# danshapero/sigma

Hardware: AMD Instinct MI355X
Metric: SpMV GB/s (achieved HBM) + CG iters/sec on 5-pt Laplacian, N=1e7 (higher is better)
Workload: dtype f64; 1 GPU; 5-point 2D Poisson CSR, 3162x3162 rows per GPU (rank 0: n=9998244, nnz=49978572), fp64 SpMV y=A*x; rows_per_gpu=9998244, nnz_per_gpu=49978572, parallelism=row-partition x1, matrix_resident_bytes_per_gpu=479920788, reference_layout_bytes_per_gpu=639735844, full=False

## Files before the change

include/sigma_hip.h:

```cpp
#ifndef SIGMA_HIP_H
#define SIGMA_HIP_H

#include <stddef.h>
#include <stdint.h>

#ifdef __cplusplus
extern "C" {
#endif

typedef struct sgm_mat_s *sgm_mat;
typedef struct sgm_pc_s *sgm_pc;
typedef struct sgm_solver_s *sgm_solver;
typedef struct sgm_comm_s *sgm_comm;

enum {
    SGM_OK = 0,
    SGM_ERR_BAD_ARG = 1,
    SGM_ERR_DIMS = 2,
    SGM_ERR_HIP = 3,
    SGM_ERR_RCCL = 4,
    SGM_ERR_NOT_CONVERGED = 5,
    SGM_ERR_NO_DEVICE = 6,
    SGM_ERR_ALLOC = 7,
    SGM_ERR_UNSUPPORTED = 8
// ... 50 lines not shown
int sgm_mat_get_entries(sgm_mat A, int64_t m, const int32_t *i, const int32_t *j, double *z_out, int where);
int sgm_mat_zero(sgm_mat A);
int sgm_mat_scalar_multiply(sgm_mat A, double alpha);
int sgm_mat_add_matrix(sgm_mat A, sgm_mat B, const double *alpha_or_null);
int sgm_edit_plan_create(sgm_edit_plan *out, sgm_mat A, int64_t m, const int32_t *i, const int32_t *j, int where);
int sgm_edit_plan_apply(sgm_edit_plan plan, sgm_mat A, const double *z, int mode, int zero_first, int where);
int sgm_edit_plan_info(sgm_edit_plan plan, int64_t *out4);
int sgm_edit_plan_destroy(sgm_edit_plan plan);
int sgm_edit_locate_host(int32_t nrow, int32_t ncol, const int32_t *ptr_1based, const int32_t *node_1based, int64_t m,
                         const int32_t *i, const int32_t *j, int64_t *hit_off, int32_t *hit_slot, int64_t capacity,
                         int64_t *needed, int64_t *first_missing);
int sgm_composite_create(sgm_mat *out, int32_t nrb, int32_t ncb, const int32_t *row_ptr_1based,
                         const int32_t *col_ptr_1based, const sgm_mat *blocks);
int sgm_mat_info(sgm_mat A, int32_t *nrow, int32_t *ncol, int64_t *nnz, int32_t *fmt,
                 int64_t *x_len );
int sgm_graph_bfs_order(sgm_mat A, int32_t *p_out);
int sgm_graph_greedy_coloring(sgm_mat A, int32_t *colors_out, int32_t *num_colors);
int sgm_graph_greedy_color_order(sgm_mat A, int32_t *p_out, int32_t *ptrs_out, int32_t ptrs_len,
                                 int32_t *num_colors);
int sgm_mat_left_permute(sgm_mat A, const int32_t *p, int where);
int sgm_mat_right_permute(sgm_mat A, const int32_t *p, int where);
int sgm_mat_kernel(sgm_mat A, char *buf, int len);
int sgm_mat_footprint(sgm_mat A, int64_t *resident_bytes, int64_t *matvec_bytes);
int sgm_mat_destroy(sgm_mat A);

int sgm_dot(int64_t n, const double *a, const double *b, double *result, int where);
int sgm_axpy(int64_t n, double alpha, const double *x, double *y, int where);

int sgm_pc_create(sgm_pc *out, int32_t kind );
int sgm_jacobi_create(sgm_pc *out, sgm_mat A);
int sgm_ildu0_create(sgm_pc *out, sgm_mat A);
int sgm_pc_setup(sgm_pc pc, sgm_mat A);
int sgm_pc_apply(sgm_pc pc, const double *r, double *z, int where);
int sgm_pc_get(sgm_pc pc, const char *name, void *out_host, size_t bytes, size_t *needed);
int sgm_pc_info(sgm_pc pc, int32_t part, int32_t *out4, double *est_us, char *path_name, int len);
int sgm_pc_destroy(sgm_pc pc);

int sgm_mg_create(sgm_pc *out, int32_t ncoarse, const sgm_mat *P ,
                  double omega, int32_t nu_pre, int32_t nu_post, int32_t coarse_sweeps);
int sgm_mg_level_matrix(sgm_pc pc, int32_t level, sgm_mat *borrowed);

int sgm_cg_create(sgm_solver *out, double tolerance);
int sgm_bicgstab_create(sgm_solver *out, double tolerance);
int sgm_gmres_create(sgm_solver *out, double tolerance, int32_t restart);
int sgm_solver_setup(sgm_solver s, sgm_mat A);
int sgm_solver_set_max_iter(sgm_solver s, int64_t max_iter );
// ... 64 lines not shown
```

sigma_amd/__init__.py:

```python
from __future__ import annotations

import ctypes as C
import os

import numpy as np

_HERE = os.path.dirname(os.path.abspath(__file__))
LIB_PATH = os.path.join(_HERE, "libsigma_hip.so")

SGM_HOST, SGM_DEVICE = 0, 1
FMT_CSR, FMT_ELL = 1, 2

_lib = None


class SigmaError(RuntimeError):

    def __init__(self, code, msg):
        super().__init__(f"[sigma_hip status {code}] {msg}")
        self.code = code


def build(force=False):
    import subprocess
# ... 198 lines not shown
        _ck(lib().sgm_graph_greedy_color_order(self._h, p.ctypes.data_as(C.c_void_p), ptrs.ctypes.data_as(C.c_void_p),
                                               C.c_int32(len(ptrs)), C.byref(nc)))
        return p, ptrs[:nc.value + 1].copy(), nc.value

    def left_permute(self, p):
        pp, w, _k = _arg(p, np.int32)
        _ck(lib().sgm_mat_left_permute(self._h, pp, C.c_int(w)))

    def right_permute(self, p):
        pp, w, _k = _arg(p, np.int32)
        _ck(lib().sgm_mat_right_permute(self._h, pp, C.c_int(w)))

    def set_option(self, name, value):
        if hasattr(self, "_build"):
            self._build()
        _ck(lib().sgm_mat_set_option(self._h, name.encode(), C.c_int(int(value))))
        return self

    @property
    def kernel(self):
        buf = C.create_string_buffer(64)
        _ck(lib().sgm_mat_kernel(self._h, buf, C.c_int(64)))
        return buf.value.decode()

    def set_solver(self, solver):
        self.solver = solver
        solver.setup(self)

    def set_preconditioner(self, pc):
        self.pc = pc
        pc.setup(self)

    def solve(self, x, b):
        if self.solver is None:
            raise SigmaError(1, "A%solve: no solver set (linear_operator_interface.f90:213-233)")
        return self.solver.solve(self, x, b, self.pc)

    def get(self, name, dtype):
        need = C.c_size_t(0)
        _ck(lib().sgm_mat_get(self._h, name.encode(), None, C.c_size_t(0), C.byref(need)))
        out = np.zeros(need.value // np.dtype(dtype).itemsize, dtype)
        _ck(lib().sgm_mat_get(self._h, name.encode(), C.c_void_p(out.ctypes.data), C.c_size_t(out.nbytes), None))
        return out

    def _triples(self, i, j, z=None):
        if not (_is_torch(i) or _is_torch(j) or (z is not None and _is_torch(z))):
# ... 831 lines not shown
```

sigma_amd/csrc/sgm_internal.hpp:

```cpp
#pragma once
#include <hip/hip_runtime.h>

#include <cstdarg>
#include <cstdint>
#include <cstdio>
#include <cstring>
#include <string>
#include <atomic>
#include <utility>
#include <vector>

#include "../../include/sigma_hip.h"

namespace sgm {

extern std::string g_err;
int fail(int code, const char *fmt, ...);

#define SGM_HIP(call)                                                              \
    do {                                                                           \
        hipError_t e__ = (call);                                                   \
        if (e__ != hipSuccess)                                                     \
            return sgm::fail(SGM_ERR_HIP, "%s:%d: %s -> %s", __FILE__, __LINE__,   \
                             #call, hipGetErrorString(e__));                       \
// ... 95 lines not shown
inline int vec_grid(int64_t n)
{
    int64_t g = (n + 4 * kBlock - 1) / (4 * kBlock);
    if (g < 1) g = 1;
    if (g > 2048) g = 2048;
    return (int)g;
}

struct ScalarRef {
    const double *ptr;
    int count;
};

struct HaloNbr {
    int peer = -1;
    int32_t send_count = 0;
    int32_t *send_idx = nullptr;
    double *send_buf = nullptr;
    int32_t recv_offset = 0;
    int32_t recv_count = 0;
};

struct SliceSched { int32_t *tab = nullptr; int32_t lo = 0, hi = 0, grid = 0, iters = 0, band = 0; };

struct Part {
    MatOptions opt = g_opt.mat;
    int32_t n = 0;
    int32_t ncol_own = 0;
    int32_t n_halo = 0;
    int32_t int_lo = 0, int_hi = 0;
    int64_t nnz = 0;
    int64_t row_begin = 0;
    int32_t *rowptr = nullptr;
    int32_t *col = nullptr;
    double *val = nullptr;
    uint8_t *code = nullptr;
    int32_t *dict = nullptr;
    int32_t ndict = 0;
    int32_t dict_reach = 0;
    int32_t max_row = 0;
    double *sval = nullptr;
    uint32_t *scode = nullptr;
    int32_t *scol = nullptr;
    uint8_t *sbcode = nullptr;
    bool lean = false;
    double *sl_val = nullptr;
    int32_t *sl_col = nullptr;
    uint16_t *sl_perm = nullptr;
    int64_t *sl_off = nullptr;
    int64_t sl_total = 0;
    int32_t *sl_win0 = nullptr;
    int32_t sl_gs = 1;
    int32_t sl_span = 0;
    int32_t sw = 0;
    int32_t sched_period = 0;
    mutable SliceSched sched[3];
    mutable int nsched = 0;
    const int32_t *run_sched = nullptr;
    int32_t run_iters = 0;
    int32_t max_d = 0;
    int32_t *ecol = nullptr;
    double *eval = nullptr;
    int32_t *edeg = nullptr;
    uint8_t *ecode = nullptr;
    int32_t emdp = 0;
    int32_t *cb_perm = nullptr;
    double *cb_sval = nullptr;
    uint16_t *cb_lcol = nullptr;
    int32_t *cb_bstart = nullptr;
    uint16_t *cb_lpos = nullptr;
    void *cb_fdesc = nullptr;
    double *cb_P = nullptr;
    int32_t cb_cols = 0, cb_nb = 0, cb_R = 0, cb_ntiles = 0, cb_chunks = 0;
    int32_t cb_maxd = 0;
    int64_t cb_count = 0;
    double col_spread = -1.0;
    std::vector<HaloNbr> nbrs;
    double *xext = nullptr;
    int dot_grid_override = 0;
    int64_t xlen() const { return (int64_t)ncol_own + n_halo; }
};

// ... 81 lines not shown
struct SpmvDots {
    const double *const *w = nullptr;
    double *const *part_wy = nullptr;
    double *const *part_yy = nullptr;
};
int spmv_parts(sgm_mat A, const double *const *x, double *const *y, bool add,
               const SpmvDots *dots, const int *flag_done, int *grid_out, int gen = 0x7fffffff,
               bool chain = false, bool halo_ready = false);

int build_csr_part(Part &p, int32_t n, int32_t ncol_own, int32_t n_halo, int64_t nnz,
                   const int32_t *ptr1, const int32_t *node1, const double *val, int where, bool validate = true);
int clone_csr_plain(sgm_mat A, sgm_mat *out);
int color_order_device(sgm_mat A, int32_t **dp, std::vector<int32_t> &ptrs);
int diag_block_plain(const Part &p, sgm_mat *out);
void part_kernel_name(const Part &p, int fmt, char *name, size_t len);
int permuted_part(const Part &p, const int32_t *p1_dev, Part &q, const int32_t *hmap_dev = nullptr,
                  const std::vector<int32_t *> *send_order = nullptr);
int halo_attach_order(const Part &p, const int32_t *p1_dev, const std::vector<std::pair<int32_t, int32_t>> &segments,
                      std::vector<int32_t> &hmap_host);
int exchange_halo_orders(sgm_mat A, const std::vector<int32_t> &mine, std::vector<int32_t *> &out);
int spmv_grid(const Part &p, bool whole = false);
int matvec_plain(sgm_mat A, const double *x, double *y);
int csr_need_arrays(const Part &p);
int ensure_transpose(sgm_mat A);
void csr_release_arrays(const Part &p);

struct Slab3;
int slab3_build(Slab3 **out, int32_t n, const std::vector<int32_t> &Lptr, const std::vector<int32_t> &Lnode,
                const std::vector<int32_t> &Uptr, const std::vector<int32_t> &Unode, const int32_t *dLptr, const int32_t *dLnode,
                const int32_t *dUptr, const int32_t *dUnode);
int slab3_refresh(Slab3 *S, const double *Lval, const double *Uval, const double *D);
void slab3_apply(const Slab3 *S, const double *r, double *z, const int *flag, int spin_limit, int32_t *sticky);
void slab3_lower_result(const Slab3 *S, double *dst);
int slab_dims_device(int32_t n, const int32_t *dptr, const int32_t *dnode, bool lower, int32_t *w, int32_t *h);
void slab3_dims(const Slab3 *S, int32_t *w, int32_t *h);
int slab3_aborted(const Slab3 *S, int32_t *abL, int32_t *abU);
void slab3_info(const Slab3 *S, int32_t out[6]);
int slab3_clocks(const Slab3 *S, std::vector<long long> &out);
void slab3_free(Slab3 *S);

}

#if defined(__HIPCC__)
namespace sgm {

template <int CTRL>
// ... 114 lines not shown
```

sigma_amd/csrc/sgm_layouts.hip:

```cpp
#include "sgm_spmv_select.hpp"

namespace sgm {

__global__ void k_dec1(int32_t *a, int64_t n)
{
    int64_t i = (int64_t)blockIdx.x * blockDim.x + threadIdx.x;
    const int64_t stride = (int64_t)gridDim.x * blockDim.x;
    for (; i < n; i += stride) a[i] -= 1;
}

__global__ void k_check_ptr1(const int32_t *__restrict__ ptr1, int64_t n, int64_t nnz, unsigned long long *bad)
{
    int64_t i = (int64_t)blockIdx.x * blockDim.x + threadIdx.x;
    const int64_t stride = (int64_t)gridDim.x * blockDim.x;
    for (; i <= n; i += stride) {
        const int32_t a = ptr1[i];
        bool ok = true;
        if (i == 0) ok = a == 1;
        if (i < n) ok = ok && ptr1[i + 1] >= a;
        else ok = ok && (int64_t)a - 1 == nnz;
        if (!ok) atomicMin(bad, (unsigned long long)i);
    }
}

// ... 237 lines not shown
        hipLaunchKernelGGL(k_sl_unpack, dim3((unsigned)std::min<int64_t>(((int64_t)p.n + 255) / 256, 4096)), dim3(256), 0, st, p.n, p.sw,
                           (const int32_t *)p.rowptr, (const uint32_t *)p.scode, (const int32_t *)p.dict, (const double *)p.sval,
                           mk_col ? p.col : nullptr, mk_val ? p.val : nullptr, mk_code ? p.code : nullptr);
    SGM_HIP(hipGetLastError());
    SGM_HIP(hipStreamSynchronize(st));
    return SGM_OK;
}
int lean_val_buffer(Part &p)
{
    if (!p.lean || p.val) return SGM_OK;
    SGM_TRY(dalloc(&p.val, (size_t)p.nnz + 2));
    SGM_HIP(hipMemsetAsync(p.val + p.nnz, 0, 2 * sizeof(double), g_rt.stream));
    return SGM_OK;
}
void csr_release_arrays(const Part &cp)
{
    Part &p = const_cast<Part &>(cp);
    if (!p.lean || !lean_applies(p)) return;
    (void)hipStreamSynchronize(g_rt.stream);
    dfree(p.val); dfree(p.col); dfree(p.code);
    p.val = nullptr; p.col = nullptr; p.code = nullptr;
}

int pack_sliced(Part &p)
{
    if (p.sl_val && p.n > 0) {
        const int64_t nch = (((int64_t)p.n + kSlRows - 1) / kSlRows) * (kSlRows / kSellChunk);
        hipLaunchKernelGGL(k_sell_fill, dim3((unsigned)std::min<int64_t>((nch + 3) / 4, 65536)), dim3(256), 0, g_rt.stream, p.n,
                           (const int32_t *)p.rowptr, (const int32_t *)nullptr, (const double *)p.val, (const int64_t *)p.sl_off,
                           (const uint16_t *)p.sl_perm, (int32_t *)nullptr, p.sl_val);
        SGM_HIP(hipGetLastError());
    }
    if ((!p.scode && !p.scol && !p.sbcode) || p.n == 0) return SGM_OK;
    const int64_t nsl = ((int64_t)p.n + kSlRows - 1) / kSlRows;
    if (p.ecol)
        hipLaunchKernelGGL(k_sl_pack_ell, dim3((unsigned)std::min<int64_t>(nsl, 65536)), dim3(256), 0, g_rt.stream, p.n, p.sw,
                           p.max_d, (const double *)p.eval, p.sval);
    else
        hipLaunchKernelGGL(k_sl_pack, dim3((unsigned)std::min<int64_t>(nsl, 65536)), dim3(256), 0, g_rt.stream, p.n, p.sw,
                           (const int32_t *)p.rowptr, (const double *)p.val, p.sval);
    SGM_HIP(hipGetLastError());
    return SGM_OK;
}

__global__ void k_fill32(int64_t n, int32_t *a, int32_t v)
{
    int64_t i = (int64_t)blockIdx.x * blockDim.x + threadIdx.x;
    const int64_t stride = (int64_t)gridDim.x * blockDim.x;
    for (; i < n; i += stride) a[i] = v;
}

constexpr int kDictSlots = 1024;
constexpr int32_t kDictEmpty = INT32_MIN;
__global__ __launch_bounds__(256) void k_dict_collect(int32_t n, const int32_t *__restrict__ rowptr, const int32_t *__restrict__ col,
                                                      int32_t *table, int *count, int *max_row)
{
    constexpr int kLocal = 512;
    __shared__ int32_t ltab[kLocal];
    __shared__ int lcount;
    for (int t = threadIdx.x; t < kLocal; t += 256) ltab[t] = kDictEmpty;
    if (threadIdx.x == 0) lcount = 0;
    __syncthreads();
    int mr = 0;
    int32_t mine[8];
// ... 226 lines not shown
                           reinterpret_cast<int32_t *>(p.scode), (int32_t)-1);
        p.sw = W;
    }
    hipLaunchKernelGGL(k_dict_encode, dim3(grid), dim3(256), 0, st, n, (const int32_t *)p.rowptr, (const int32_t *)p.col,
                       (const int32_t *)p.dict, p.ndict, p.code, sliced ? p.scode : nullptr);
    SGM_HIP(hipGetLastError());
    if (sliced) SGM_TRY(pack_sliced(p));
    int Wb = 0;
#define PICK(WW) if (!Wb && p.max_row <= WW) Wb = WW;
    SGM_SLB_WIDTHS(PICK)
#undef PICK
    const int Wc = (Wb + 7) / 8 * 8;
    if (!sliced && p.opt.csr_sliced && Wb && p.ndict <= 255 && p.max_row > 8 && (double)Wb * n <= 1.35 * (double)nnz) {
        rows_padded = ((size_t)n + kSlRows - 1) / kSlRows * kSlRows;
        SGM_TRY(dalloc(&p.sbcode, rows_padded * Wc));
        SGM_TRY(dalloc(&p.sval, rows_padded * Wb));
        p.sw = Wb;
        hipLaunchKernelGGL(k_slb_pack_codes, dim3((unsigned)std::min<size_t>(rows_padded / kSlRows, 65536)), dim3(256), 0, st, n, Wb,
                           (const int32_t *)p.rowptr, (const uint8_t *)p.code, p.sbcode);
        SGM_HIP(hipGetLastError());
        SGM_TRY(pack_sliced(p));
    }
    SGM_HIP(hipStreamSynchronize(st));
    if (p.scode || p.sbcode) SGM_TRY(detect_sched_period_csr(p, dict));
    if (!p.scode && !p.sbcode) {
        SGM_TRY(build_sell(p));
        if (p.sl_val) {
            dfree(p.code); dfree(p.dict);
            p.code = nullptr; p.dict = nullptr;
            p.ndict = 0; p.dict_reach = 0;
        }
    }
    csr_go_lean(p);
    return SGM_OK;
}

__global__ __launch_bounds__(256) void k_ell_dict_collect(int32_t n, int32_t max_d, const int32_t *__restrict__ ecol, int32_t *table,
                                                          int *count)
{
    constexpr int kLocal = 512;
    __shared__ int32_t ltab[kLocal];
    __shared__ int lcount;
    for (int t = threadIdx.x; t < kLocal; t += 256) ltab[t] = kDictEmpty;
    if (threadIdx.x == 0) lcount = 0;
    __syncthreads();
    int32_t mine[8];
// ... 197 lines not shown
    int rc = dalloc(&q.rowptr, (size_t)p.n + 1);
    if (rc == SGM_OK) rc = dalloc(&q.col, (size_t)p.nnz + 4);
    if (rc == SGM_OK) rc = dalloc(&q.val, (size_t)p.nnz + 2);
    if (rc != SGM_OK) { sgm_mat_destroy(C); return rc; }
    (void)hipMemcpyAsync(q.rowptr, p.rowptr, ((size_t)p.n + 1) * 4, hipMemcpyDeviceToDevice, st);
    (void)hipMemsetAsync(q.col + p.nnz, 0, 16, st);
    (void)hipMemsetAsync(q.val + p.nnz, 0, 16, st);
    if (p.nnz) {
        (void)hipMemcpyAsync(q.col, p.col, (size_t)p.nnz * 4, hipMemcpyDeviceToDevice, st);
        (void)hipMemcpyAsync(q.val, p.val, (size_t)p.nnz * 8, hipMemcpyDeviceToDevice, st);
    }
    if (hipStreamSynchronize(st) != hipSuccess || hipGetLastError() != hipSuccess) { sgm_mat_destroy(C); return fail(SGM_ERR_HIP, "clone_csr_plain: copy failed"); }
    *out = C;
    return SGM_OK;
}

int rebuild_csr_formats(Part &p)
{
    SGM_TRY(csr_need_arrays(p));
    p.lean = false;
    dfree(p.code); dfree(p.dict); dfree(p.sval); dfree(p.scode); dfree(p.scol); dfree(p.sbcode);
    p.code = nullptr; p.dict = nullptr; p.sval = nullptr; p.scode = nullptr; p.scol = nullptr; p.sbcode = nullptr;
    free_sell(p);
    free_ell_colblock(p);
    p.ndict = 0; p.dict_reach = 0; p.sw = 0; p.max_row = 0; p.sched_period = 0;
    free_slice_sched(p);
    return build_offset_dict(p, nullptr, nullptr);
}
int rebuild_ell_formats(Part &p)
{
    dfree(p.ecode); dfree(p.dict); dfree(p.sval); dfree(p.scode);
    p.ecode = nullptr; p.dict = nullptr; p.dict_reach = 0; p.emdp = 0; p.sval = nullptr; p.scode = nullptr; p.sw = 0; p.sched_period = 0;
    free_slice_sched(p);
    SGM_TRY(build_ell_offset_dict(p));
    SGM_TRY(build_ell_colblock(p));
    return refresh_ell_colblock_values(p);
}
int sgm_invalidate_transpose(sgm_mat A)
{
    if (A->T) { sgm_mat_destroy(A->T); A->T = nullptr; }
    dfree(A->tperm);
    A->tperm = nullptr;
    A->t_stale = true;
    return SGM_OK;
}

void free_part(Part &p)
{
    dfree(p.rowptr); dfree(p.col); dfree(p.val); dfree(p.code); dfree(p.dict); dfree(p.sval); dfree(p.scode); dfree(p.scol); dfree(p.sbcode); dfree(p.ecol); dfree(p.eval); dfree(p.edeg); dfree(p.ecode); dfree(p.xext);
    for (auto &nb : p.nbrs) { dfree(nb.send_idx); dfree(nb.send_buf); }
    free_slice_sched(p);
    free_ell_colblock(p);
    free_sell(p);
    p = Part();
}

}
```

sigma_amd/csrc/sgm_mat.hip:

```cpp
#include "sgm_spmv_select.hpp"

namespace sgm {

struct Staged {
    double *dev = nullptr;
    bool owned = false;
    ~Staged() { if (owned) dfree(dev); }
};
int stage_in(Staged &s, const double *v, int64_t n, int where, bool copy)
{
    if (where == SGM_DEVICE && (reinterpret_cast<uintptr_t>(v) & 15) == 0) {
        s.dev = const_cast<double *>(v);
        return SGM_OK;
    }
    SGM_TRY(dalloc(&s.dev, (size_t)n));
    s.owned = true;
    if (copy)
        SGM_HIP(hipMemcpyAsync(s.dev, v, (size_t)n * 8,
                               where == SGM_HOST ? hipMemcpyHostToDevice : hipMemcpyDeviceToDevice,
                               g_rt.stream));
    return SGM_OK;
}
int stage_out(const Staged &s, double *v, int64_t n, int where)
{
// ... 371 lines not shown
    if (!mat_option_field(probe, name)) return fail(SGM_ERR_BAD_ARG, "sgm_mat_set_option: '%s' is not a matrix option", name);
    if (A->fmt == SGM_FMT_COMPOSITE) {
        for (sgm_mat_s *B : A->blocks)
            if (B) SGM_TRY(sgm_mat_set_option(B, name, value));
        return SGM_OK;
    }
    const bool cb_shape = !strcmp(name, "ell_colblock_cols") || !strcmp(name, "ell_colblock_rows");
    for (Part &p : A->parts) {
        int *f = mat_option_field(p.opt, name);
        const int old = *f;
        *f = v;
        if (old == v) continue;
        if ((p.ecol || (!p.lean && p.rowptr && p.col && p.val && p.n_halo == 0 && !p.sval && !p.sl_val)) &&
            (cb_shape || (!strcmp(name, "ell_colblock") && ((old != 0) != (v != 0) || v == 2 || old == 2)))) {
            SGM_TRY(build_ell_colblock(p));
            SGM_TRY(refresh_ell_colblock_values(p));
            SGM_HIP(hipStreamSynchronize(g_rt.stream));
        }
        if (!strcmp(name, "csr_lean") && !p.ecol) {
            if (v == 0) { SGM_TRY(csr_need_arrays(p)); p.lean = false; }
            else csr_go_lean(p);
        }
        if (!strcmp(name, "slice_sched")) free_slice_sched(p);
    }
    if (A->T) SGM_TRY(sgm_mat_set_option(A->T, name, value));
    return SGM_OK;
}

int sgm_mat_matvec(sgm_mat A, const double *x, double *y, int where)
{
    return matvec_impl(A, x, y, where, false);
}

int sgm_mat_matvec_add(sgm_mat A, const double *x, double *y, int where)
{
    return matvec_impl(A, x, y, where, true);
}

int sgm_composite_create(sgm_mat *out, int32_t nrb, int32_t ncb, const int32_t *row_ptr, const int32_t *col_ptr,
                         const sgm_mat *blocks)
{
    SGM_TRY(require_init());
    if (!out || nrb < 1 || ncb < 1 || !row_ptr || !col_ptr || !blocks)
        return fail(SGM_ERR_BAD_ARG, "sgm_composite_create: bad argument");
    sgm_mat A = new sgm_mat_s;
    A->fmt = SGM_FMT_COMPOSITE;
// ... 159 lines not shown
}
extern "C" {

int sgm_mat_kernel(sgm_mat A, char *buf, int len)
{
    if (!A || !buf || len < 1) return fail(SGM_ERR_BAD_ARG, "sgm_mat_kernel: bad argument");
    char name[64];
    if (A->fmt == SGM_FMT_COMPOSITE) snprintf(name, sizeof name, "composite");
    else part_kernel_name(A->parts[0], A->fmt, name, sizeof name);
    snprintf(buf, (size_t)len, "%s", name);
    return SGM_OK;
}

static int64_t part_resident_bytes(const Part &p)
{
    int64_t b = 0;
    const int64_t nsl = ((int64_t)p.n + kSlRows - 1) / kSlRows;
    if (p.rowptr) b += 4 * ((int64_t)p.n + 1);
    if (p.col) b += 4 * (p.nnz + 4);
    if (p.val) b += 8 * (p.nnz + 2);
    if (p.code) b += p.nnz + 16;
    if (p.dict) b += 4 * 256;
    if (p.sval) b += 8 * nsl * kSlRows * p.sw;
    if (p.scode) b += 4 * nsl * kSlRows;
    if (p.scol) b += 4 * nsl * kSlRows * p.sw;
    if (p.sbcode) b += nsl * kSlRows * ((p.sw + 7) / 8 * 8);
    if (p.sl_val) b += 12 * p.sl_total + 2 * nsl * kSlRows + 8 * (nsl * (kSlRows / kSellChunk) + 1);
    if (p.ecol) b += 4 * (int64_t)p.n * p.max_d;
    if (p.eval) b += 8 * (int64_t)p.n * p.max_d;
    if (p.edeg) b += 4 * (int64_t)p.n;
    if (p.ecode) b += (int64_t)p.n * p.emdp;
    if (p.xext) b += 8 * p.xlen();
    b += ell_colblock_resident_bytes(p);
    for (const auto &nb : p.nbrs) b += (int64_t)nb.send_count * (nb.send_buf ? 12 : 4);
    return b;
}
static int64_t part_matvec_bytes(const sgm_mat_s *A, const Part &p)
{
    const int64_t nsl = ((int64_t)p.n + kSlRows - 1) / kSlRows;
    int64_t m;
    if (A->fmt == SGM_FMT_ELL) {
        if (use_ell_colblock(p)) return ell_colblock_matvec_bytes(p);
        if (use_sliced_ell(p)) m = nsl * kSlRows * (8 * (int64_t)p.sw + 4);
        else if (p.ecode && p.opt.ell_offset_dict) m = (int64_t)p.n * (8 * (int64_t)p.max_d + p.emdp);
        else m = 12 * (int64_t)p.n * p.max_d;
    } else if (use_ell_colblock(p)) return ell_colblock_matvec_bytes(p);
    else if (use_sliced(p)) m = nsl * kSlRows * (8 * (int64_t)p.sw + 4);
    else if (use_slicedb(p)) m = nsl * kSlRows * (8 * (int64_t)p.sw + (p.sw + 7) / 8 * 8);
    else if (use_sliced32(p)) m = nsl * kSlRows * 12 * (int64_t)p.sw;
    else if (use_sell(p)) {
        m = 12 * p.sl_total + 2 * nsl * kSlRows + 8 * nsl * (kSlRows / kSellChunk);
        if (p.sl_win0 && p.opt.csr_xwindow)
            return m + ((nsl + p.sl_gs - 1) / p.sl_gs) * (8 * (int64_t)p.sl_span + 4) + 8 * (int64_t)p.n;
    }
    else if (use_offset_dict(p)) m = 9 * p.nnz + 4 * ((int64_t)p.n + 1);
    else m = 12 * p.nnz + 4 * ((int64_t)p.n + 1);
    return m + 8 * p.xlen() + 8 * (int64_t)p.n;
}

int sgm_mat_footprint(sgm_mat A, int64_t *resident_bytes, int64_t *matvec_bytes)
{
    if (!A) return fail(SGM_ERR_BAD_ARG, "sgm_mat_footprint: null matrix");
    int64_t res = 0, mv = 0;
    if (A->fmt == SGM_FMT_COMPOSITE) {
        for (sgm_mat C : A->blocks) {
            if (!C) continue;
            int64_t r = 0, m = 0;
            SGM_TRY(sgm_mat_footprint(C, &r, &m));
            mv += m + 8 * (int64_t)C->nrow;
        }
        mv += 8 * (int64_t)A->nrow;
    } else {
        for (const Part &p : A->parts) { res += part_resident_bytes(p); mv += part_matvec_bytes(A, p); }
        if (A->T) { int64_t r = 0; SGM_TRY(sgm_mat_footprint(A->T, &r, nullptr)); res += r + 4 * A->nnz; }
    }
    if (resident_bytes) *resident_bytes = res;
    if (matvec_bytes) *matvec_bytes = mv;
    return SGM_OK;
}

int sgm_mat_destroy(sgm_mat A)
{
    if (!A) return SGM_OK;
    for (auto &p : A->parts) free_part(p);
    if (A->T) sgm_mat_destroy(A->T);
    dfree(A->tperm);
    alg_plan_free(A->alg);
    delete A;
    return SGM_OK;
}

}
```

sigma_amd/csrc/sgm_runtime.hip:

```cpp
#include "sgm_internal.hpp"

#include <algorithm>

namespace sgm {

std::string g_err;
Runtime g_rt;
Options g_opt;
Heartbeat g_hb;
extern int g_force_collectives;

int fail(int code, const char *fmt, ...)
{
    char buf[1024];
    va_list ap;
    va_start(ap, fmt);
    vsnprintf(buf, sizeof buf, fmt, ap);
    va_end(ap);
    g_err = buf;
    return code;
}

bool trace_on()
{
// ... 69 lines not shown
    SGM_OPT(mat, ell_colblock_rows) SGM_OPT(mat, slice_sched) SGM_OPT(mat, coloring_pass)
    return nullptr;
}
int *solver_option_field(SolverOptions &o, const char *name)
{
    SGM_OPT(solver, cg_small) SGM_OPT(solver, bicgstab_small) SGM_OPT(solver, krylov_graph) SGM_OPT(solver, dot_order)
    SGM_OPT(solver, gmres_cgs2) SGM_OPT(solver, dist_halo_fused) SGM_OPT(solver, coop_spin_limit) SGM_OPT(solver, cg_coop_variant)
    SGM_OPT(solver, reorder_solve)
    return nullptr;
}
int *pc_option_field(PcOptions &o, const char *name)
{
    SGM_OPT(pc, ildu_strips) SGM_OPT(pc, ildu_rows) SGM_OPT(pc, pipeline_spin_limit) SGM_OPT(pc, ildu_reorder)
    return nullptr;
}
#undef SGM_OPT

int normalise_option(const char *name, int value, int *out)
{
    int v = value;
    if (!strcmp(name, "ell_colblock_cols")) v = std::min(kEllcbMaxCols, std::max(2, value)) & ~1;
    else if (!strcmp(name, "ell_colblock_rows")) v = value == 512 ? 512 : value == 256 ? 256 : 0;
    else if (!strcmp(name, "ildu_reorder")) v = value != 0;
    else if (!strcmp(name, "csr_sell")) v = value < 0 ? 0 : value > 2 ? 2 : value;
    else if (!strcmp(name, "csr_lean") || !strcmp(name, "csr_xwindow")) v = value != 0;
    else if (!strcmp(name, "slice_sched")) v = value <= 0 ? 0 : value == 1 ? 1 : std::max(4, value);
    else if (!strcmp(name, "krylov_graph")) v = value <= 0 ? 0 : value == 1 ? 1 : std::max(16, (value + 15) / 16 * 16);
    else if (!strcmp(name, "cg_small")) v = std::max(0, value);
    else if (!strcmp(name, "dist_halo_fused") || !strcmp(name, "reorder_solve")) v = value < 0 ? 0 : value > 2 ? 2 : value;
    else if (!strcmp(name, "coop_spin_limit")) v = std::max(0, value);
    else if (!strcmp(name, "gmres_cgs2")) v = value != 0;
    else if (!strcmp(name, "cg_coop_variant")) {
        const int r = value & 15;
        if (value < 0 || value > 31 || (r != 0 && r != 1 && r != 2 && r != 4 && r != 8))
            return fail(SGM_ERR_BAD_ARG, "option cg_coop_variant: rows per thread 0 (by size), 1, 2, 4 or 8, + 16 = no one-XCD variant");
    }
    else if (!strcmp(name, "coloring_pass")) v = value < 0 ? 0 : value > 2 ? 2 : value;
    else if (!strcmp(name, "pipeline_spin_limit")) v = std::max(0, value);
    else if (!strcmp(name, "dot_order") && value != 0 && value != 1)
        return fail(SGM_ERR_BAD_ARG, "option dot_order is 0 (tree) or 1 (the reference's sequential order)");
    *out = v;
    return SGM_OK;
}

}

// ... 121 lines not shown
```

sigma_amd/csrc/sgm_spmv.hip:

```cpp
#include "sgm_spmv_select.hpp"
#include "sgm_plan_host.hpp"

namespace sgm {




__device__ inline int64_t rowblock_of(int it, int b, int grid, int64_t nrb = 0, int mode = 1)
{
    const int per = grid >> 3;
    if (mode == 2) {
        const int64_t chunk = (nrb + 7) / 8;
        const int64_t local = (int64_t)it * per + (b >> 3);
        return local < chunk ? (int64_t)(b & 7) * chunk + local : nrb;
    }
    return (int64_t)it * grid + (int64_t)(b & 7) * per + (b >> 3);
}


template <class T>
__device__ inline T ld_stream(const T *p, bool nt)
{
    return nt ? __builtin_nontemporal_load(p) : *p;
}
// ... 329 lines not shown
#pragma unroll
                for (int u = 0; u < U; ++u)
                    if (u < cnt) z = z + vv[u] * xv[u];
                k += cnt;
            }
        }
        if (row < n) {
            const double yi = ADD ? (chain ? z : y0 + z) : 0.0 + z;
            __builtin_nontemporal_store(yi, y + row);
            if (DOT_W) dwy += w[row] * yi;
            if (DOT_YY) dyy += yi * yi;
        }
    }
    if (DOT_W) {
        const double t = block_sum<BLOCK>(dwy, red);
        if (tid == 0) part_wy[blockIdx.x] = t;
    }
    if (DOT_YY) {
        const double t = block_sum<BLOCK>(dyy, red);
        if (tid == 0) part_yy[blockIdx.x] = t;
    }
}

template <int W, bool ADD, bool DOT_W, bool DOT_YY>
__global__ __launch_bounds__(256) void k_csr_sl(
    int32_t n, const uint32_t *__restrict__ scode, const int32_t *__restrict__ dict,
    const double *__restrict__ sval, const double *__restrict__ x, double *__restrict__ y,
    const double *__restrict__ w, double *__restrict__ part_wy, double *__restrict__ part_yy,
    const int *__restrict__ flag_done, int gen, int remap, const int32_t *__restrict__ sched, int sched_iters)
{
    constexpr int BLOCK = 256;
    __shared__ int32_t dl[16];
    __shared__ double red[BLOCK / 64];
    const int st = flag_done ? *flag_done : 0;
    const int tid = threadIdx.x;
    const bool chain = (remap & 256) != 0;
    const int32_t dv = tid < 16 ? dict[tid] : 0;
    const int64_t nsl = ((int64_t)n + kSlRows - 1) / kSlRows;
    double dwy = 0.0, dyy = 0.0;

    int64_t first = blockIdx.x;
    if ((remap & 255) >= 3) {
        const int G = (remap & 255) == 3 ? 8 : (remap & 255) == 4 ? 2 : (remap & 255) == 6 ? 64 : (remap & 255) == 7 ? 128 : 32;
        const int xcd = blockIdx.x & 7, loc = blockIdx.x >> 3;
        first = (int64_t)(loc / G) * (8 * G) + xcd * G + loc % G;
    }
    int64_t sl = sched ? sched[blockIdx.x] : first;
    int sit = 0;
    u32x2 cw = {0xffffffffu, 0xffffffffu};
    f64x2 v[W];
    auto load_slice = [&](int64_t s_) {
        const int32_t row_ = (int32_t)(s_ * kSlRows) + 2 * tid;
        cw = __builtin_nontemporal_load(reinterpret_cast<const u32x2 *>(scode + row_));
        const f64x2 *vb = reinterpret_cast<const f64x2 *>(sval + s_ * (int64_t)(W * kSlRows)) + tid;
#pragma unroll
        for (int u = 0; u < W; ++u) v[u] = __builtin_nontemporal_load(vb + u * BLOCK);
// ... 521 lines not shown
    } while (0)
#define LV(B, T)                                \
    if (c.block == B && tile == T) {            \
        if (w && pyy) L(B, T, true, true);      \
        else if (w) L(B, T, true, false);       \
        else if (pyy) L(B, T, false, true);     \
        else L(B, T, false, false);             \
        return;                                 \
    }
    SGM_DO_VARIANTS(LV)
#undef LV
#undef L
}

template <bool ADD>
static void launch_csr_sl(const Part &p, int grid, const double *x, double *y, const double *w,
                          double *pwy, double *pyy, const int *flag, int gen)
{
    const SpmvCfg &c = spmv_cfg();
    hipStream_t st = g_rt.stream;
    int mode = c.remap == 1 ? ((grid <= kMaxGrid / 2 || (int64_t)p.n < (int64_t)32768 * kSlRows) ? 5 : 0) : (c.remap >= 3 ? c.remap : 0);
    if (mode >= 3 && grid % (8 * (mode == 3 ? 8 : mode == 4 ? 2 : mode == 6 ? 64 : mode == 7 ? 128 : 32)) != 0) mode = 0;
#define L(WW, DW, DY)                                                                                   \
    hipLaunchKernelGGL((k_csr_sl<WW, ADD, DW, DY>), dim3(grid), dim3(256), 0, st, p.n, p.scode, p.dict, \
                       p.sval, x, y, w, pwy, pyy, flag, gen, mode | g_launch_flags, p.run_sched, p.run_iters)
#define LV(WW)                                \
    if (p.sw == WW) {                         \
        if (w && pyy) L(WW, true, true);      \
        else if (w) L(WW, true, false);       \
        else if (pyy) L(WW, false, true);     \
        else L(WW, false, false);             \
        return;                               \
    }
    SGM_SL_WIDTHS(LV)
#undef LV
#undef L
}

template <bool ADD>
static void launch_csr_sl32(const Part &p, int grid, const double *x, double *y, const double *w,
                            double *pwy, double *pyy, const int *flag, int gen)
{
    hipStream_t st = g_rt.stream;
    const SpmvCfg &c = spmv_cfg();
    int mode = c.remap == 1 ? ((grid <= kMaxGrid / 2 || (int64_t)p.n < (int64_t)32768 * kSlRows) ? 5 : 0) : (c.remap >= 3 ? c.remap : 0);
    if (mode >= 3 && grid % (8 * (mode == 3 ? 8 : mode == 4 ? 2 : mode == 6 ? 64 : mode == 7 ? 128 : 32)) != 0) mode = 0;
#define L(WW, DW, DY)                                                                                     \
    hipLaunchKernelGGL((k_csr_sl32<WW, ADD, DW, DY>), dim3(grid), dim3(256), 0, st, p.n, p.scol, p.sval, x, y, \
// ... 198 lines not shown
    ss.tab = d; ss.iters = iters;
    return &ss;
}
void free_slice_sched(Part &p)
{
    for (int i = 0; i < p.nsched; ++i) { dfree(p.sched[i].tab); p.sched[i] = SliceSched(); }
    p.nsched = 0;
}

static void launch_range(sgm_mat A, const Part &p, const RowRange &r, const double *x, double *y, bool add,
                         const double *w, double *pwy, double *pyy, const int *flag_done, int gen)
{
    Part v;
    v.opt = p.opt;
    v.n = r.hi - r.lo;
    v.nnz = (int64_t)((double)p.nnz * v.n / (p.n > 0 ? p.n : 1));
    v.n_halo = p.n_halo; v.ncol_own = p.ncol_own;
    v.rowptr = p.rowptr + r.lo; v.col = p.col; v.val = p.val; v.code = p.code; v.dict = p.dict;
    v.max_row = p.max_row;
    const bool sliced = use_sliced(p), slicedb = !sliced && use_slicedb(p), sliced32 = !sliced && !slicedb && use_sliced32(p);
    if (sliced || slicedb)
        if (const SliceSched *ss = slice_sched(p, r.lo, r.hi, r.grid)) { v.run_sched = ss->tab; v.run_iters = ss->iters; }
    if (sliced) { v.sval = p.sval + (int64_t)r.lo * p.sw; v.scode = p.scode + r.lo; v.sw = p.sw; }
    if (slicedb) { v.sval = p.sval + (int64_t)r.lo * p.sw; v.sbcode = p.sbcode + (int64_t)r.lo * ((p.sw + 7) / 8 * 8); v.sw = p.sw; }
    if (sliced32) { v.sval = p.sval + (int64_t)r.lo * p.sw; v.scol = p.scol + (int64_t)r.lo * p.sw; v.sw = p.sw; }
    const bool sell = !sliced && !slicedb && !sliced32 && use_sell(p);
    if (sell) {
        v.sl_val = p.sl_val; v.sl_col = p.sl_col;
        v.sl_off = p.sl_off + r.lo / kSellChunk; v.sl_perm = p.sl_perm + r.lo;
        v.sl_gs = p.sl_gs;
        v.sl_win0 = p.sl_win0 ? p.sl_win0 + r.lo / (kSlRows * p.sl_gs) : nullptr; v.sl_span = p.sl_span;
    }
    const bool dict = use_offset_dict(p);
    const double *xs = dict ? x + r.lo : x;
    double *ys = y + r.lo;
    const double *ws = w ? w + r.lo : nullptr;
    double *pw = pwy ? pwy + r.part_off : nullptr, *py = pyy ? pyy + r.part_off : nullptr;
    if (sliced) {
        if (add) launch_csr_sl<true>(v, r.grid, xs, ys, ws, pw, py, flag_done, gen);
        else launch_csr_sl<false>(v, r.grid, xs, ys, ws, pw, py, flag_done, gen);
    } else if (slicedb) {
        if (add) launch_csr_slb<true>(v, r.grid, xs, ys, ws, pw, py, flag_done, gen);
        else launch_csr_slb<false>(v, r.grid, xs, ys, ws, pw, py, flag_done, gen);
    } else if (sliced32) {
        if (add) launch_csr_sl32<true>(v, r.grid, x, ys, ws, pw, py, flag_done, gen);
        else launch_csr_sl32<false>(v, r.grid, x, ys, ws, pw, py, flag_done, gen);
// ... 163 lines not shown
```

Before: 6465 GB/s.

## Replace per-entry sliced CSR values with a verified 16-entry value table

Adds a GPU check-and-merge pass that tests whether every nonzero sharing a 4-bit sliced-CSR code has the same value. If so, the SpMV kernel switches to a TAB variant that reads coefficients from a small table in shared memory instead of streaming sval, and prefetches codes a few slices ahead. The aim is to remove the dominant value traffic from each matvec. The cost is an extra verification kernel and host synchronisation at setup. The reported matvec byte count now drops to the code stream only, which changes how the GB/s figure is computed.

```diff
diff --git a/include/sigma_hip.h b/include/sigma_hip.h
--- a/include/sigma_hip.h
+++ b/include/sigma_hip.h
@@ -96,6 +96,7 @@
 int sgm_mat_right_permute(sgm_mat A, const int32_t *p, int where);
 int sgm_mat_kernel(sgm_mat A, char *buf, int len);
 int sgm_mat_footprint(sgm_mat A, int64_t *resident_bytes, int64_t *matvec_bytes);
+int sgm_mat_value_table(sgm_mat A, int *state);
 int sgm_mat_destroy(sgm_mat A);
 
 int sgm_dot(int64_t n, const double *a, const double *b, double *result, int where);
diff --git a/sigma_amd/__init__.py b/sigma_amd/__init__.py
--- a/sigma_amd/__init__.py
+++ b/sigma_amd/__init__.py
@@ -244,6 +244,14 @@
         buf = C.create_string_buffer(64)
         _ck(lib().sgm_mat_kernel(self._h, buf, C.c_int(64)))
         return buf.value.decode()
+
+    @property
+    def value_table(self):
+        if hasattr(self, "_build"):
+            self._build()
+        s = C.c_int(0)
+        _ck(lib().sgm_mat_value_table(self._h, C.byref(s)))
+        return s.value
 
     def set_solver(self, solver):
         self.solver = solver
diff --git a/sigma_amd/csrc/sgm_internal.hpp b/sigma_amd/csrc/sgm_internal.hpp
--- a/sigma_amd/csrc/sgm_internal.hpp
+++ b/sigma_amd/csrc/sgm_internal.hpp
@@ -141,6 +141,18 @@
 };
 
 struct SliceSched { int32_t *tab = nullptr; int32_t lo = 0, hi = 0, grid = 0, iters = 0, band = 0; };
+
+constexpr int64_t kValueTableAutoBytes = (int64_t)256 << 20;
+inline int value_table_mode(const MatOptions &o) { return o.csr_sliced == 1 ? 1 : o.csr_sliced == 2 ? 2 : 0; }
+struct ValueTable {
+    double *tab = nullptr;
+    int32_t *verdict = nullptr;
+    hipEvent_t ev = nullptr;
+    int state = -1;
+    int32_t gen = 0;
+    bool pending = false;
+};
+constexpr int64_t kValueTableBytes = 16 * 8 + 2 * 4;
 
 struct Part {
     MatOptions opt = g_opt.mat;
@@ -177,6 +189,8 @@
     mutable int nsched = 0;
     const int32_t *run_sched = nullptr;
     int32_t run_iters = 0;
+    ValueTable *vt = nullptr;
+    const double *run_vtab = nullptr;
     int32_t max_d = 0;
     int32_t *ecol = nullptr;
     double *eval = nullptr;
@@ -304,6 +318,10 @@
 int spmv_grid(const Part &p, bool whole = false);
 int matvec_plain(sgm_mat A, const double *x, double *y);
 int csr_need_arrays(const Part &p);
+bool value_table_wanted(const Part &p);
+int verify_value_table(Part &p);
+void adopt_value_table(const Part &p);
+bool value_table_on(const Part &p);
 int ensure_transpose(sgm_mat A);
 void csr_release_arrays(const Part &p);
 
diff --git a/sigma_amd/csrc/sgm_layouts.hip b/sigma_amd/csrc/sgm_layouts.hip
--- a/sigma_amd/csrc/sgm_layouts.hip
+++ b/sigma_amd/csrc/sgm_layouts.hip
@@ -283,6 +283,153 @@
     p.val = nullptr; p.col = nullptr; p.code = nullptr;
 }
 
+constexpr int kVtGrid = 1024, kVtSlot = 17;
+__global__ __launch_bounds__(256) void k_vt_check(int32_t n, int W, const uint32_t *__restrict__ scode, const double *__restrict__ sval,
+                                                  unsigned long long *__restrict__ slots)
+{
+    typedef unsigned long long u64x2 __attribute__((ext_vector_type(2)));
+    __shared__ unsigned long long cand[16];
+    __shared__ unsigned present, bad;
+    const int tid = threadIdx.x;
+    if (tid < 16) cand[tid] = 0ull;
+    if (tid == 0) { present = 0u; bad = 0u; }
+    __syncthreads();
+    const int64_t nsl = ((int64_t)n + kSlRows - 1) / kSlRows;
+    bool mybad = false;
+    for (int64_t s = blockIdx.x; s < nsl; s += gridDim.x) {
+        const u32x2 cw = *reinterpret_cast<const u32x2 *>(scode + s * kSlRows + 2 * tid);
+        const u64x2 *vb = reinterpret_cast<const u64x2 *>(sval + s * (int64_t)W * kSlRows) + tid;
+        u64x2 v[8];
+#pragma unroll
+        for (int u = 0; u < 8; ++u) v[u] = u < W ? vb[u * (kSlRows / 2)] : u64x2{0ull, 0ull};
+        const unsigned have = present;
+        unsigned mine = 0u;
+#pragma unroll
+        for (int u = 0; u < 8; ++u) {
+            const uint32_t ca = (cw.x >> (4 * u)) & 15u, cb = (cw.y >> (4 * u)) & 15u;
+            if (u < W && ca != 15u && !((have >> ca) & 1u)) { cand[ca] = v[u].x; mine |= 1u << ca; }
+            if (u < W && cb != 15u && !((have >> cb) & 1u)) { cand[cb] = v[u].y; mine |= 1u << cb; }
+        }
+        __syncthreads();
+        if (mine) atomicOr(&present, mine);
+#pragma unroll
+        for (int u = 0; u < 8; ++u) {
+            const uint32_t ca = (cw.x >> (4 * u)) & 15u, cb = (cw.y >> (4 * u)) & 15u;
+            if (u < W && ca != 15u && cand[ca] != v[u].x) mybad = true;
+            if (u < W && cb != 15u && cand[cb] != v[u].y) mybad = true;
+        }
+        __syncthreads();
+    }
+    if (mybad) atomicOr(&bad, 1u);
+    __syncthreads();
+    unsigned long long *slot = slots + (int64_t)blockIdx.x * kVtSlot;
+    if (tid < 16) slot[tid] = ((present >> tid) & 1u) ? cand[tid] : 0ull;
+    if (tid == 0) slot[16] = (unsigned long long)present | ((unsigned long long)bad << 16);
+}
+__global__ __launch_bounds__(kVtGrid) void k_vt_merge(int nslots, const unsigned long long *__restrict__ slots, unsigned long long *__restrict__ out,
+                                                      int32_t gen)
+{
+    __shared__ int first[16];
+    __shared__ unsigned long long cand[16];
+    __shared__ unsigned fail;
+    const int b = threadIdx.x;
+    if (b < 16) { first[b] = INT32_MAX; cand[b] = 0ull; }
+    if (b == 0) fail = 0u;
+    unsigned long long v[15], m = 0ull;
+    if (b < nslots) {
+        m = slots[(int64_t)b * kVtSlot + 16];
+#pragma unroll
+        for (int c = 0; c < 15; ++c) v[c] = slots[(int64_t)b * kVtSlot + c];
+    }
+    __syncthreads();
+    if (m >> 16) atomicOr(&fail, 1u);
+#pragma unroll
+    for (int c = 0; c < 15; ++c)
+        if ((m >> c) & 1ull) atomicMin(&first[c], b);
+    __syncthreads();
+#pragma unroll
+    for (int c = 0; c < 15; ++c)
+        if (((m >> c) & 1ull) && first[c] == b) cand[c] = v[c];
+    __syncthreads();
+    bool bad = false;
+#pragma unroll
+    for (int c = 0; c < 15; ++c)
+        if (((m >> c) & 1ull) && cand[c] != v[c]) bad = true;
+    if (bad) atomicOr(&fail, 1u);
+    __syncthreads();
+    if (b < 16) out[b] = cand[b];
+    if (b == 0) {
+        int32_t *vd = reinterpret_cast<int32_t *>(out + 16);
+        vd[0] = fail ? 0 : 1;
+        vd[1] = gen;
+    }
+}
+
+bool value_table_wanted(const Part &p)
+{
+    if (!p.scode || !p.sval || !p.dict || p.ecol || p.scol || p.sbcode || p.sw > 8 || p.n <= 0 || !value_table_mode(p.opt)) return false;
+    if (value_table_mode(p.opt) == 2) return true;
+    const int64_t nsl = ((int64_t)p.n + kSlRows - 1) / kSlRows;
+    return 8 * (int64_t)p.sw * nsl * kSlRows > kValueTableAutoBytes;
+}
+static void free_value_table(Part &p)
+{
+    if (!p.vt) return;
+    dfree(p.vt->tab);
+    if (p.vt->verdict) (void)hipHostFree(p.vt->verdict);
+    if (p.vt->ev) (void)hipEventDestroy(p.vt->ev);
+    delete p.vt;
+    p.vt = nullptr;
+}
+int verify_value_table(Part &p)
+{
+    static unsigned long long *scratch = nullptr;
+    static int scratch_dev = -1;
+    if (scratch_dev != g_rt.device) {
+        dfree(scratch); scratch = nullptr; scratch_dev = -1;
+        SGM_TRY(dalloc(&scratch, (size_t)kVtGrid * kVtSlot));
+        scratch_dev = g_rt.device;
+    }
+    hipStream_t st = g_rt.stream;
+    if (!p.vt) {
+        ValueTable *t = new ValueTable;
+        p.vt = t;
+        SGM_TRY(dalloc(&t->tab, (size_t)kValueTableBytes / 8));
+        SGM_HIP(hipMemsetAsync(t->tab, 0, (size_t)kValueTableBytes, st));
+        SGM_HIP(hipHostMalloc((void **)&t->verdict, 2 * sizeof(int32_t), hipHostMallocDefault));
+        t->verdict[0] = 0; t->verdict[1] = -1;
+        SGM_HIP(hipEventCreateWithFlags(&t->ev, hipEventDisableTiming));
+    }
+    ValueTable *t = p.vt;
+    const int64_t nsl = ((int64_t)p.n + kSlRows - 1) / kSlRows;
+    const int grid = (int)std::min<int64_t>(nsl, kVtGrid);
+    hipLaunchKernelGGL(k_vt_check, dim3(grid), dim3(256), 0, st, p.n, p.sw, (const uint32_t *)p.scode, (const double *)p.sval, scratch);
+    hipLaunchKernelGGL(k_vt_merge, dim3(1), dim3(kVtGrid), 0, st, grid, (const unsigned long long *)scratch,
+                       reinterpret_cast<unsigned long long *>(t->tab), t->gen);
+    SGM_HIP(hipGetLastError());
+    SGM_HIP(hipMemcpyAsync(t->verdict, t->tab + 16, 2 * sizeof(int32_t), hipMemcpyDeviceToHost, st));
+    SGM_HIP(hipEventRecord(t->ev, st));
+    t->pending = true;
+    return SGM_OK;
+}
+void adopt_value_table(const Part &p)
+{
+    ValueTable *t = p.vt;
+    if (!t || !t->pending) return;
+    hipStreamCaptureStatus cs = hipStreamCaptureStatusNone;
+    if (hipStreamIsCapturing(g_rt.stream, &cs) != hipSuccess) { (void)hipGetLastError(); return; }
+    if (cs != hipStreamCaptureStatusNone) return;
+    if (hipEventQuery(t->ev) != hipSuccess) { (void)hipGetLastError(); return; }
+    t->pending = false;
+    if (t->verdict[1] == t->gen) t->state = t->verdict[0] ? 1 : 0;
+}
+bool value_table_on(const Part &p)
+{
+    if (!p.vt || !use_sliced(p) || !value_table_wanted(p)) return false;
+    if (p.vt->pending) adopt_value_table(p);
+    return p.vt->state == 1;
+}
+
 int pack_sliced(Part &p)
 {
     if (p.sl_val && p.n > 0) {
@@ -301,6 +448,8 @@
         hipLaunchKernelGGL(k_sl_pack, dim3((unsigned)std::min<int64_t>(nsl, 65536)), dim3(256), 0, g_rt.stream, p.n, p.sw,
                            (const int32_t *)p.rowptr, (const double *)p.val, p.sval);
     SGM_HIP(hipGetLastError());
+    if (p.vt) { p.vt->state = -1; p.vt->gen += 1; p.vt->pending = false; }
+    if (value_table_wanted(p)) SGM_TRY(verify_value_table(p));
     return SGM_OK;
 }
 
@@ -573,6 +722,7 @@
         SGM_TRY(pack_sliced(p));
     }
     SGM_HIP(hipStreamSynchronize(st));
+    adopt_value_table(p);
     if (p.scode || p.sbcode) SGM_TRY(detect_sched_period_csr(p, dict));
     if (!p.scode && !p.sbcode) {
         SGM_TRY(build_sell(p));
@@ -816,6 +966,7 @@
     dfree(p.code); dfree(p.dict); dfree(p.sval); dfree(p.scode); dfree(p.scol); dfree(p.sbcode);
     p.code = nullptr; p.dict = nullptr; p.sval = nullptr; p.scode = nullptr; p.scol = nullptr; p.sbcode = nullptr;
     free_sell(p);
+    free_value_table(p);
     free_ell_colblock(p);
     p.ndict = 0; p.dict_reach = 0; p.sw = 0; p.max_row = 0; p.sched_period = 0;
     free_slice_sched(p);
@@ -846,6 +997,7 @@
     free_slice_sched(p);
     free_ell_colblock(p);
     free_sell(p);
+    free_value_table(p);
     p = Part();
 }
 
diff --git a/sigma_amd/csrc/sgm_mat.hip b/sigma_amd/csrc/sgm_mat.hip
--- a/sigma_amd/csrc/sgm_mat.hip
+++ b/sigma_amd/csrc/sgm_mat.hip
@@ -417,6 +417,11 @@
             else csr_go_lean(p);
         }
         if (!strcmp(name, "slice_sched")) free_slice_sched(p);
+        if (!strcmp(name, "csr_sliced") && value_table_wanted(p) && !(p.vt && (p.vt->pending || p.vt->state >= 0))) {
+            SGM_TRY(verify_value_table(p));
+            SGM_HIP(hipStreamSynchronize(g_rt.stream));
+            adopt_value_table(p);
+        }
     }
     if (A->T) SGM_TRY(sgm_mat_set_option(A->T, name, value));
     return SGM_OK;
@@ -622,6 +627,7 @@
     if (p.code) b += p.nnz + 16;
     if (p.dict) b += 4 * 256;
     if (p.sval) b += 8 * nsl * kSlRows * p.sw;
+    if (p.vt) b += kValueTableBytes;
     if (p.scode) b += 4 * nsl * kSlRows;
     if (p.scol) b += 4 * nsl * kSlRows * p.sw;
     if (p.sbcode) b += nsl * kSlRows * ((p.sw + 7) / 8 * 8);
@@ -645,7 +651,7 @@
         else if (p.ecode && p.opt.ell_offset_dict) m = (int64_t)p.n * (8 * (int64_t)p.max_d + p.emdp);
         else m = 12 * (int64_t)p.n * p.max_d;
     } else if (use_ell_colblock(p)) return ell_colblock_matvec_bytes(p);
-    else if (use_sliced(p)) m = nsl * kSlRows * (8 * (int64_t)p.sw + 4);
+    else if (use_sliced(p)) m = value_table_on(p) ? nsl * kSlRows * 4 : nsl * kSlRows * (8 * (int64_t)p.sw + 4);
     else if (use_slicedb(p)) m = nsl * kSlRows * (8 * (int64_t)p.sw + (p.sw + 7) / 8 * 8);
     else if (use_sliced32(p)) m = nsl * kSlRows * 12 * (int64_t)p.sw;
     else if (use_sell(p)) {
@@ -679,6 +685,21 @@
     return SGM_OK;
 }
 
+int sgm_mat_value_table(sgm_mat A, int *state)
+{
+    if (!A || !state) return fail(SGM_ERR_BAD_ARG, "sgm_mat_value_table: null argument");
+    *state = 0;
+    if (A->fmt != SGM_FMT_CSR) return SGM_OK;
+    int sliced = 0, on = 0;
+    for (const Part &p : A->parts) {
+        if (!use_sliced(p)) continue;
+        ++sliced;
+        if (value_table_on(p)) ++on;
+    }
+    *state = sliced > 0 && on == sliced;
+    return SGM_OK;
+}
+
 int sgm_mat_destroy(sgm_mat A)
 {
     if (!A) return SGM_OK;
diff --git a/sigma_amd/csrc/sgm_runtime.hip b/sigma_amd/csrc/sgm_runtime.hip
--- a/sigma_amd/csrc/sgm_runtime.hip
+++ b/sigma_amd/csrc/sgm_runtime.hip
@@ -115,6 +115,7 @@
     if (!strcmp(name, "ell_colblock_cols")) v = std::min(kEllcbMaxCols, std::max(2, value)) & ~1;
     else if (!strcmp(name, "ell_colblock_rows")) v = value == 512 ? 512 : value == 256 ? 256 : 0;
     else if (!strcmp(name, "ildu_reorder")) v = value != 0;
+    else if (!strcmp(name, "csr_sliced")) v = value < 0 ? 0 : value > 3 ? 3 : value;
     else if (!strcmp(name, "csr_sell")) v = value < 0 ? 0 : value > 2 ? 2 : value;
     else if (!strcmp(name, "csr_lean") || !strcmp(name, "csr_xwindow")) v = value != 0;
     else if (!strcmp(name, "slice_sched")) v = value <= 0 ? 0 : value == 1 ? 1 : std::max(4, value);
diff --git a/sigma_amd/csrc/sgm_spmv.hip b/sigma_amd/csrc/sgm_spmv.hip
--- a/sigma_amd/csrc/sgm_spmv.hip
+++ b/sigma_amd/csrc/sgm_spmv.hip
@@ -375,7 +375,10 @@
     }
 }
 
-template <int W, bool ADD, bool DOT_W, bool DOT_YY>
+#ifndef SGM_VTAB_AHEAD
+#define SGM_VTAB_AHEAD 2
+#endif
+template <int W, bool ADD, bool DOT_W, bool DOT_YY, bool TAB = false>
 __global__ __launch_bounds__(256) void k_csr_sl(
     int32_t n, const uint32_t *__restrict__ scode, const int32_t *__restrict__ dict,
     const double *__restrict__ sval, const double *__restrict__ x, double *__restrict__ y,
@@ -385,6 +388,94 @@
     constexpr int BLOCK = 256;
     __shared__ int32_t dl[16];
     __shared__ double red[BLOCK / 64];
+    if (TAB) {
+        constexpr int kAhead = SGM_VTAB_AHEAD;
+        __shared__ double tl[16];
+        const int st = flag_done ? *flag_done : 0;
+        const int tid = threadIdx.x;
+        const bool chain = (remap & 256) != 0;
+        const int32_t dv = tid < 16 ? dict[tid] : 0;
+        const double tv = tid < 16 ? sval[tid] : 0.0;
+        const int64_t nsl = ((int64_t)n + kSlRows - 1) / kSlRows;
+        double dwy = 0.0, dyy = 0.0;
+        int64_t seq = blockIdx.x;
+        if ((remap & 255) >= 3) {
+            const int G = (remap & 255) == 3 ? 8 : (remap & 255) == 4 ? 2 : (remap & 255) == 6 ? 64 : (remap & 255) == 7 ? 128 : 32;
+            const int xcd = blockIdx.x & 7, loc = blockIdx.x >> 3;
+            seq = (int64_t)(loc / G) * (8 * G) + xcd * G + loc % G;
+        }
+        int sit = 0;
+        int64_t sq[kAhead + 1];
+        u32x2 cq[kAhead + 1];
+        bool open = true;
+        auto request = [&](int64_t s_, int k) {
+            open = open && s_ >= 0 && s_ < nsl;
+            sq[k] = open ? s_ : -1;
+            cq[k] = u32x2{0xffffffffu, 0xffffffffu};
+            if (open) cq[k] = __builtin_nontemporal_load(reinterpret_cast<const u32x2 *>(scode + ((int32_t)(s_ * kSlRows) + 2 * tid)));
+        };
+        auto following = [&]() -> int64_t {
+            if (!open) return -1;
+            if (sched) { ++sit; return sit < sched_iters ? sched[(int64_t)sit * gridDim.x + blockIdx.x] : -1; }
+            seq += gridDim.x;
+            return seq;
+        };
+        request(sched ? sched[blockIdx.x] : seq, 0);
+#pragma unroll
+        for (int k = 1; k <= kAhead; ++k) request(following(), k);
+        if (st && gen >= st) return;
+        if (tid < 16) { dl[tid] = dv; tl[tid] = tv; }
+        __syncthreads();
+        while (sq[0] >= 0) {
+            const u32x2 cw = cq[0];
+            const int32_t row = (int32_t)(sq[0] * kSlRows) + 2 * tid;
+#pragma unroll
+            for (int k = 0; k < kAhead; ++k) { sq[k] = sq[k + 1]; cq[k] = cq[k + 1]; }
+            request(following(), kAhead);
+            f64x2 y0 = {0.0, 0.0};
+            if (ADD) {
+                if (row + 1 < n) y0 = *reinterpret_cast<const f64x2 *>(y + row);
+                else if (row < n) y0.x = y[row];
+            }
+            double xa[W], xb[W];
+#pragma unroll
+            for (int u = 0; u < W; ++u) {
+                const uint32_t ca = (cw.x >> (4 * u)) & 15u, cb = (cw.y >> (4 * u)) & 15u;
+                xa[u] = ca != 15u ? x[row + dl[ca]] : 0.0;
+                xb[u] = cb != 15u ? x[row + 1 + dl[cb]] : 0.0;
+            }
+            f64x2 z;
+            z.x = (ADD && chain) ? y0.x : 0.0;
+            z.y = (ADD && chain) ? y0.y : 0.0;
+#pragma unroll
+            for (int u = 0; u < W; ++u) {
+                const uint32_t ca = (cw.x >> (4 * u)) & 15u, cb = (cw.y >> (4 * u)) & 15u;
+                if (ca != 15u) z.x = z.x + tl[ca] * xa[u];
+                if (cb != 15u) z.y = z.y + tl[cb] * xb[u];
+            }
+            f64x2 yi;
+            yi.x = ADD ? (chain ? z.x : y0.x + z.x) : 0.0 + z.x;
+            yi.y = ADD ? (chain ? z.y : y0.y + z.y) : 0.0 + z.y;
+            if (row + 1 < n) {
+                __builtin_nontemporal_store(yi, reinterpret_cast<f64x2 *>(y + row));
+                if (DOT_W) { const f64x2 wv = *reinterpret_cast<const f64x2 *>(w + row); dwy += wv.x * yi.x; dwy += wv.y * yi.y; }
+                if (DOT_YY) { dyy += yi.x * yi.x; dyy += yi.y * yi.y; }
+            } else if (row < n) {
+                __builtin_nontemporal_store(yi.x, y + row);
+                if (DOT_W) dwy += w[row] * yi.x;
+                if (DOT_YY) dyy += yi.x * yi.x;
+            }
+        }
+        if (DOT_W) {
+            const double t = block_sum<BLOCK>(dwy, red);
+            if (tid == 0) part_wy[blockIdx.x] = t;
+        }
+        if (DOT_YY) {
+            const double t = block_sum<BLOCK>(dyy, red);
+            if (tid == 0) part_yy[blockIdx.x] = t;
+        }
+        return;
+    }
     const int st = flag_done ? *flag_done : 0;
     const int tid = threadIdx.x;
     const bool chain = (remap & 256) != 0;
@@ -952,8 +1043,14 @@
     int mode = c.remap == 1 ? ((grid <= kMaxGrid / 2 || (int64_t)p.n < (int64_t)32768 * kSlRows) ? 5 : 0) : (c.remap >= 3 ? c.remap : 0);
     if (mode >= 3 && grid % (8 * (mode == 3 ? 8 : mode == 4 ? 2 : mode == 6 ? 64 : mode == 7 ? 128 : 32)) != 0) mode = 0;
 #define L(WW, DW, DY)                                                                                   \
-    hipLaunchKernelGGL((k_csr_sl<WW, ADD, DW, DY>), dim3(grid), dim3(256), 0, st, p.n, p.scode, p.dict, \
-                       p.sval, x, y, w, pwy, pyy, flag, gen, mode | g_launch_flags, p.run_sched, p.run_iters)
+    do {                                                                                                \
+        if (p.run_vtab)                                                                                 \
+            hipLaunchKernelGGL((k_csr_sl<WW, ADD, DW, DY, true>), dim3(grid), dim3(256), 0, st, p.n, p.scode, p.dict, \
+                               p.run_vtab, x, y, w, pwy, pyy, flag, gen, mode | g_launch_flags, p.run_sched, p.run_iters); \
+        else                                                                                            \
+            hipLaunchKernelGGL((k_csr_sl<WW, ADD, DW, DY>), dim3(grid), dim3(256), 0, st, p.n, p.scode, p.dict, \
+                               p.sval, x, y, w, pwy, pyy, flag, gen, mode | g_launch_flags, p.run_sched, p.run_iters); \
+    } while (0)
 #define LV(WW)                                \
     if (p.sw == WW) {                         \
         if (w && pyy) L(WW, true, true);      \
@@ -1198,6 +1295,7 @@
     if (sliced || slicedb)
         if (const SliceSched *ss = slice_sched(p, r.lo, r.hi, r.grid)) { v.run_sched = ss->tab; v.run_iters = ss->iters; }
     if (sliced) { v.sval = p.sval + (int64_t)r.lo * p.sw; v.scode = p.scode + r.lo; v.sw = p.sw; }
+    if (sliced && value_table_on(p)) v.run_vtab = p.vt->tab;
     if (slicedb) { v.sval = p.sval + (int64_t)r.lo * p.sw; v.sbcode = p.sbcode + (int64_t)r.lo * ((p.sw + 7) / 8 * 8); v.sw = p.sw; }
     if (sliced32) { v.sval = p.sval + (int64_t)r.lo * p.sw; v.scol = p.scol + (int64_t)r.lo * p.sw; v.sw = p.sw; }
     const bool sell = !sliced && !slicedb && !sliced32 && use_sell(p);
```

Measured after the change: 4603 GB/s. -28.8%, worse.
